# GrokImageCompression/Grok

Measured on NVIDIA H100. Metric: Mpixels/s encode+decode 8K RGB 12-bit HTJ2K; DWT HBM GB/s vs roofline, higher is better.
Workload: dtype i32

## Files before the change

grok_b200/csrc/b2k_internal.h:

```cpp
#pragma once
#include <stdint.h>
#include <stddef.h>
#include <atomic>
#include <functional>
#include <cuda_runtime.h>
#include "../../include/grok_b200.h"

#define B2K_WARPS_PER_CTA 4

struct DeviceOnce
{
  std::atomic<uint64_t> done{0};
  template <class F> void run(F&& f)
  {
    int dev = 0;
    cudaGetDevice(&dev);
    const uint64_t bit = 1ull << (dev & 63);
    if(!(done.load(std::memory_order_acquire) & bit))
    {
      f();
      done.fetch_or(bit, std::memory_order_release);
    }
  }
};
// ... 9 lines not shown
  int32_t shift[3];
  int32_t lo[3], hi[3];
  uint16_t nstrips, nsegs, strip_w, pairs_per_seg;
  uint8_t first_level;
  uint8_t comp0;
  uint8_t pad[2];
};

struct HtBlockDesc
{
  void* coef;
  uint32_t pitch;
  uint16_t w, h;
  uint8_t kmax;
  uint8_t irreversible;
  uint8_t mmsbs;
  uint8_t passes;
  float quant;
  uint32_t slot_cap;
  uint64_t slot_off;
  uint32_t length;
  uint32_t rec_off;
  uint32_t length2;
};
static_assert(sizeof(HtBlockDesc) == 56, "HtBlockDesc layout");

struct HtBlockOut
{
  uint32_t ms_len, mel_len, vlc_len, total;
};

void b2k_launch_dwt_fwd(const DwtLevelDesc* d_descs, int ndesc, int max_jobs, int nc, bool irreversible, cudaStream_t st);
void b2k_launch_dwt_inv(const DwtLevelDesc* d_descs, int ndesc, int max_jobs, int nc, bool irreversible, cudaStream_t st);
void b2k_launch_point_transform(const DwtLevelDesc* d_descs, int ndesc, uint32_t max_w, uint32_t max_h, int nc, bool irreversible,
                                bool forward, cudaStream_t st);
struct HtEncodeLimits
{
  uint32_t stage_words;
  uint32_t max_kmax;
};
uint32_t b2k_ht_encode_stage_words(uint32_t w);
void b2k_launch_ht_encode(const HtBlockDesc* d_blocks, HtBlockOut* d_out, uint8_t* d_scratch, uint32_t nblocks,
                          const HtEncodeLimits& lim, bool irreversible, cudaStream_t st);
void b2k_launch_ht_gather(const HtBlockDesc* d_blocks, const HtBlockOut* d_out, const uint64_t* d_offsets,
                          const uint8_t* d_scratch, uint8_t* d_bytes, uint32_t nblocks, uint64_t cap, cudaStream_t st);
void b2k_launch_scan_lengths(const HtBlockOut* d_out, uint64_t* d_offsets, uint32_t nblocks, cudaStream_t st);
void b2k_launch_ht_decode_refine(const HtBlockDesc* d_blocks, const uint8_t* d_bytes, const HtBlockOut* d_status,
                                 uint32_t nblocks, int stripe_causal, cudaStream_t st);
void b2k_launch_ht_decode(const HtBlockDesc* d_blocks, const uint8_t* d_bytes, uint32_t* d_recs, HtBlockOut* d_status,
                          uint32_t nblocks, uint32_t max_w, int* d_err, int irreversible, int any_refinement, cudaStream_t st);
void b2k_launch_ht_decode_vlc(const HtBlockDesc* d_blocks, const uint8_t* d_bytes, uint32_t* d_recs, HtBlockOut* d_status,
                              uint32_t nblocks, uint32_t max_w, cudaStream_t st);
void b2k_launch_ht_decode_magsgn(const HtBlockDesc* d_blocks, const uint8_t* d_bytes, const uint32_t* d_recs,
                                 const HtBlockOut* d_status, uint32_t nblocks, uint32_t max_w, int* d_err, int irreversible,
                                 int any_refinement, cudaStream_t st);
void b2k_launch_build_dec_desc(const HtBlockDesc* d_enc, const HtBlockOut* d_out, const uint64_t* d_offsets,
                               const float* d_dec_quant, HtBlockDesc* d_dec, uint32_t n, cudaStream_t st);
void b2k_launch_container_to_planes(const void* src, uint32_t spitch, uint32_t step, uint32_t sample_bytes, int32_t* const* dst, int nc,
                                    uint32_t dpitch, uint32_t w, uint32_t h, int sgnd, cudaStream_t st);
void b2k_launch_planes_to_container(const int32_t* const* src, int nc, uint32_t spitch, void* dst, uint32_t dpitch, uint32_t step,
                                    uint32_t sample_bytes, uint32_t w, uint32_t h, cudaStream_t st);
void b2k_count_launch(void);

struct b2k_host_rect
{
  const void* src;
// ... 11 lines not shown
```

grok_b200/csrc/dwt.cu:

```cuda
#include "b2k_internal.h"

namespace {

__device__ __noinline__ int mirror_rel_slow(int t, int n)
{
  if(n == 1)
    return 0;
  const int period = 2 * (n - 1);
  t %= period;
  if(t < 0)
    t += period;
  return t < n ? t : period - t;
}
__device__ __forceinline__ int mirror_rel(int t, int n)
{
  if((unsigned)t < (unsigned)n)
    return t;
  const int r = t < 0 ? -t : 2 * (n - 1) - t;
  if((unsigned)r < (unsigned)n)
    return r;
  return mirror_rel_slow(t, n);
}

__device__ __forceinline__ void load8_w32(const int32_t* __restrict__ row, int rel, int n, int (&v)[8])
// ... 11 lines not shown
#pragma unroll
    for(int i = 0; i < 8; ++i)
      v[i] = __ldg(row + mirror_rel(rel + i, n));
  }
}

__device__ __forceinline__ void load4_band(const int32_t* __restrict__ row, int k0, int kb0, int u0, int u1, int odd,
                                           int (&v)[4])
{
  const int ufirst = 2 * k0 + odd, ulast = ufirst + 6;
  const int32_t* p = row + (k0 - kb0);
  if(ufirst >= u0 && ulast < u1 && ((reinterpret_cast<uintptr_t>(p) & 15) == 0))
  {
    const int4 a = __ldg(reinterpret_cast<const int4*>(p));
    v[0] = a.x; v[1] = a.y; v[2] = a.z; v[3] = a.w;
  }
  else
  {
    const int n = u1 - u0;
#pragma unroll
    for(int i = 0; i < 4; ++i)
    {
      const int um = u0 + mirror_rel(ufirst + 2 * i - u0, n);
      v[i] = ((um & 1) == odd) ? __ldg(row + ((um >> 1) - kb0)) : 0;
    }
  }
}

struct Job
{
  int lane, ulane, jbeg, jend, wn, hn, nvalid;
  bool owner, need;
};
template <bool WHOLE>
__device__ __forceinline__ bool decode_job(const DwtLevelDesc& D, Job& J)
{
  J.lane = threadIdx.x & 31;
  const int job = blockIdx.x * B2K_WARPS_PER_CTA + (threadIdx.x >> 5);
  if(job >= (int)D.nstrips * (int)D.nsegs)
    return false;
  const int strip = job % D.nstrips, seg = job / D.nstrips;
  constexpr int halo = WHOLE ? 0 : 1;
  J.wn = D.u1 - D.u0;
  J.hn = D.v1 - D.v0;
  J.nvalid = D.strip_w >> 3;
  J.ulane = (D.u0 & ~7) + strip * (int)D.strip_w + (J.lane - halo) * 8;
  J.owner = J.lane >= halo && J.lane < J.nvalid + halo && J.ulane < D.u1;
  J.need = J.lane <= J.nvalid + halo && J.ulane < D.u1 + 8;
  const int jlo = D.v0 >> 1, jhi = (D.v1 - 1) >> 1;
  J.jbeg = jlo + seg * (int)D.pairs_per_seg;
  J.jend = min(J.jbeg + (int)D.pairs_per_seg, jhi + 1);
  return true;
}

template <int NC, int N>
__device__ __forceinline__ void rct_fwd(const DwtLevelDesc& D, int (&x)[NC][N])
{
#pragma unroll
  for(int i = 0; i < N; ++i)
  {
    if constexpr(NC == 3)
    {
      const int r = x[0][i] + D.shift[0], g = x[1][i] + D.shift[1], b = x[2][i] + D.shift[2];
      x[0][i] = ((g + g) + b + r) >> 2;
      x[1][i] = b - g;
      x[2][i] = r - g;
    }
    else
      x[0][i] += D.shift[0];
  }
}

template <int NC, int N>
__device__ __forceinline__ void ict_fwd(const DwtLevelDesc& D, const int (&x)[NC][N], float (&out)[NC][N])
{
  const float a_r = 0.299f, a_g = 0.587f, a_b = 0.114f;
  const float cb = __fdiv_rn(0.5f, __fsub_rn(1.0f, a_b)), cr = __fdiv_rn(0.5f, __fsub_rn(1.0f, a_r));
#pragma unroll
  for(int i = 0; i < N; ++i)
  {
    if constexpr(NC == 3)
    {
// ... 72 lines not shown
__device__ __forceinline__ void to_coeffs53(const DwtLevelDesc& D, int (&x)[NC][N])
{
  if(D.first_level)
    rct_fwd<NC, N>(D, x);
}

template <int NC>
__device__ __forceinline__ void to_coeffs97(const DwtLevelDesc& D, const int (&raw)[NC][8], float (&out)[NC][8])
{
  if(D.first_level)
    ict_fwd<NC>(D, raw, out);
  else
  {
#pragma unroll
    for(int c = 0; c < NC; ++c)
#pragma unroll
      for(int i = 0; i < 8; ++i)
        out[c][i] = __int_as_float(raw[c][i]);
  }
}

template <int NC>
__device__ __forceinline__ void fetch53(const DwtLevelDesc& D, const Job& J, int v, int (&out)[NC][8])
{
  fetch_int_rows<NC>(D, J, v, out);
  to_coeffs53<NC>(D, out);
}

struct GhostCol
{
  int col;
  int slot;
};
__device__ __forceinline__ GhostCol ghost_col(const DwtLevelDesc& D, const Job& J)
{
  const int x0 = J.ulane - 8 * J.lane;
  GhostCol G;
  G.slot = J.lane == 0 ? 0 : J.lane == 1 ? 1 : J.lane == 31 ? 2 : -1;
  const int x = J.lane == 0 ? x0 - 1 : J.lane == 1 ? x0 - 2 : J.lane == 31 ? x0 + 256 : J.ulane;
  G.col = mirror_rel(x - D.u0, J.wn);
  return G;
}
template <int NC>
__device__ __forceinline__ void fetch_ghost53(const DwtLevelDesc& D, const Job& J, const GhostCol& G, int v, int (&out)[NC][1])
{
  const int r = mirror_rel(v - D.v0, J.hn);
#pragma unroll
  for(int c = 0; c < NC; ++c)
    out[c][0] = __ldg(reinterpret_cast<const int32_t*>(D.in[c]) + (size_t)r * D.in_pitch + G.col);
  to_coeffs53<NC>(D, out);
}

template <int NC>
__device__ __forceinline__ void fetch97(const DwtLevelDesc& D, const Job& J, int v, float (&out)[NC][8])
{
  int raw[NC][8];
  fetch_int_rows<NC>(D, J, v, raw);
  to_coeffs97<NC>(D, raw, out);
}

struct BandGeom
{
  int x0l, x0h, y0l, y0h, snx, sny;
};
__device__ __forceinline__ BandGeom band_geom(const DwtLevelDesc& D)
{
  BandGeom g;
  g.x0l = (D.u0 + 1) >> 1;
  g.x0h = D.u0 >> 1;
  g.y0l = (D.v0 + 1) >> 1;
  g.y0h = D.v0 >> 1;
  g.snx = ((D.u1 + 1) >> 1) - g.x0l;
  g.sny = ((D.v1 + 1) >> 1) - g.y0l;
  return g;
}

struct StoreCtx
{
  unsigned mlo, mhi;
  bool vec_ll, vec_lo, vec_hi;
  int col_ll, col_lo, col_hi;
};
__device__ __forceinline__ StoreCtx store_ctx(const DwtLevelDesc& D, const Job& J, const BandGeom& g)
{
  StoreCtx s;
  s.mlo = s.mhi = 0;
  if(J.owner)
  {
#pragma unroll
    for(int i = 0; i < 4; ++i)
    {
      const int ue = J.ulane + 2 * i;
      if(ue >= D.u0 && ue < D.u1)
        s.mlo |= 1u << i;
      if(ue + 1 >= D.u0 && ue + 1 < D.u1)
        s.mhi |= 1u << i;
    }
  }
  const int k0 = J.ulane >> 1;
  s.col_ll = k0 - g.x0l;
  s.col_lo = k0 - g.x0l;
  s.col_hi = g.snx + k0 - g.x0h;
  const bool pitch_ok = ((D.ll_pitch | D.c_pitch) & 3u) == 0;
  s.vec_ll = pitch_ok && s.mlo == 0xF && (((reinterpret_cast<uintptr_t>(D.out_ll[0]) >> 2) + (unsigned)s.col_ll) & 3u) == 0;
  s.vec_lo = pitch_ok && s.mlo == 0xF && (((reinterpret_cast<uintptr_t>(D.out_c[0]) >> 2) + (unsigned)s.col_lo) & 3u) == 0;
  s.vec_hi = pitch_ok && s.mhi == 0xF && (((reinterpret_cast<uintptr_t>(D.out_c[0]) >> 2) + (unsigned)s.col_hi) & 3u) == 0;
  return s;
}
__device__ __forceinline__ void store4v(int32_t* __restrict__ p, const int (&v)[4], unsigned mask, bool vec)
{
  if(vec)
    *reinterpret_cast<int4*>(p) = make_int4(v[0], v[1], v[2], v[3]);
  else
  {
#pragma unroll
    for(int i = 0; i < 4; ++i)
      if(mask & (1u << i))
        p[i] = v[i];
  }
}
__device__ __forceinline__ void store_rows(const DwtLevelDesc& D, const BandGeom& g, const StoreCtx& S, int c, int j,
                                           bool vhigh, const int (&lo)[4], const int (&hi)[4])
{
  const int v = 2 * j + (vhigh ? 1 : 0);
  if(v < D.v0 || v >= D.v1 || (S.mlo | S.mhi) == 0)
    return;
  if(!vhigh)
  {
    const int r = j - g.y0l;
    store4v(reinterpret_cast<int32_t*>(D.out_ll[c]) + (r * (int)D.ll_pitch + S.col_ll), lo, S.mlo, S.vec_ll);
    store4v(reinterpret_cast<int32_t*>(D.out_c[c]) + (r * (int)D.c_pitch + S.col_hi), hi, S.mhi, S.vec_hi);
  }
  else
  {
    const int r = g.sny + j - g.y0h;
    int32_t* crow = reinterpret_cast<int32_t*>(D.out_c[c]) + r * (int)D.c_pitch;
    store4v(crow + S.col_lo, lo, S.mlo, S.vec_lo);
    store4v(crow + S.col_hi, hi, S.mhi, S.vec_hi);
  }
}

template <bool DEGEN = true>
__device__ __forceinline__ void hfwd53(const int (&r)[8], int g, int wn, int (&lo)[4], int (&hi)[4])
{
  const int lane = threadIdx.x & 31;
  const int g2 = __shfl_down_sync(0xffffffffu, g, 1);
  const int rn = __shfl_down_sync(0xffffffffu, r[0], 1);
  const int en = lane == 31 ? g : rn;
  hi[0] = r[1] - ((r[0] + r[2]) >> 1);
  hi[1] = r[3] - ((r[2] + r[4]) >> 1);
  hi[2] = r[5] - ((r[4] + r[6]) >> 1);
  hi[3] = r[7] - ((r[6] + en) >> 1);
  const int hp = __shfl_up_sync(0xffffffffu, hi[3], 1);
  const int dp = lane == 0 ? g - ((g2 + r[0]) >> 1) : hp;
  lo[0] = r[0] + ((dp + hi[0] + 2) >> 2);
  lo[1] = r[2] + ((hi[0] + hi[1] + 2) >> 2);
  lo[2] = r[4] + ((hi[1] + hi[2] + 2) >> 2);
  lo[3] = r[6] + ((hi[2] + hi[3] + 2) >> 2);
  if(DEGEN && wn == 1)
  {
#pragma unroll
    for(int i = 0; i < 4; ++i)
    {
      lo[i] = r[2 * i];
      hi[i] = r[2 * i + 1] << 1;
    }
  }
}

#define F97_ALPHA (-1.586134342f)
#define F97_BETA (-0.052980118f)
// ... 148 lines not shown
        mbar_fence_init();
      }
      __syncwarp();
    }
#pragma unroll
    for(int s = 0; s < DWT_STAGES - 1; ++s)
      refill(fill_bulk, fill_async, fill_side);
  }
  template <class Bulk, class Async, class Side = NoSideFill>
  __device__ __forceinline__ const uint8_t* acquire(int t, const Bulk& fill_bulk, const Async& fill_async,
                                                    const Side& fill_side = Side())
  {
    if(Stage::COOPERATIVE || bulk)
      __syncwarp();
    refill(fill_bulk, fill_async, fill_side);
    const int k = t - tfirst;
    if(bulk)
    {
      mbar_wait(bars + k % DWT_STAGES, (unsigned)((k / DWT_STAGES) & 1));
      if(Stage::GHOSTS)
        cp_async_wait<DWT_STAGES - 1>();
    }
    else
    {
      cp_async_wait<DWT_STAGES - 1>();
      if(Stage::COOPERATIVE)
        __syncwarp();
    }
    return slots + (size_t)(k % DWT_STAGES) * Stage::PAIRB;
  }
  __device__ __forceinline__ void drain() const { cp_async_wait<0>(); }
};

template <int NC, bool GHOSTS_ = false>
struct RowStage
{
  static constexpr int ROWB = 1024;
  static constexpr int BODYB = 2 * NC * ROWB;
  static constexpr bool GHOSTS = GHOSTS_;
  static constexpr int PAIRB = BODYB + (GHOSTS ? 2 * NC * 16 : 0);
  static constexpr bool COOPERATIVE = true;
  static __device__ __forceinline__ int swz(int k) { return k ^ ((k >> 3) & 1); }

  template <class MCol>
  static __device__ __forceinline__ void fill(uint8_t* stage, int which, const DwtLevelDesc& D, const Job& J, int v,
                                              bool fast, unsigned fastmask, const MCol& mcol)
  {
    const int r = mirror_rel(v - D.v0, J.hn);
    const int rel = J.ulane - D.u0;
#pragma unroll
    for(int c = 0; c < NC; ++c)
    {
      uint8_t* dst = stage + (which * NC + c) * ROWB;
      const int32_t* row = reinterpret_cast<const int32_t*>(D.in[c]) + (size_t)r * D.in_pitch;
      const int rel0 = rel - 8 * J.lane;
#pragma unroll
      for(int h = 0; h < 2; ++h)
      {
        const int k = J.lane + 32 * h;
        if((fastmask >> (k >> 1)) & 1u)
          cp_async16(dst + swz(k) * 16, row + rel0 + 4 * k);
      }
      if(J.need && !fast)
      {
        uint8_t* d0 = dst + swz(2 * J.lane) * 16;
        uint8_t* d1 = dst + swz(2 * J.lane + 1) * 16;
#pragma unroll
        for(int i = 0; i < 4; ++i)
        {
          cp_async4(d0 + 4 * i, row + mcol(i));
          cp_async4(d1 + 4 * i, row + mcol(4 + i));
        }
      }
    }
  }
  static __device__ __forceinline__ void fill_ghost(uint8_t* stage, int which, const DwtLevelDesc& D, const Job& J, int v,
                                                    const GhostCol& G)
  {
    static_assert(GHOSTS, "stage without ghost columns");
    const int r = mirror_rel(v - D.v0, J.hn);
#pragma unroll
    for(int c = 0; c < NC; ++c)
      if(G.slot >= 0)
        cp_async4(stage + BODYB + (which * NC + c) * 16 + 4 * G.slot,
                  reinterpret_cast<const int32_t*>(D.in[c]) + (size_t)r * D.in_pitch + G.col);
  }
  static __device__ __forceinline__ int2 ghost_at(const Job& J, const GhostCol& G)
  {
    return G.slot >= 0 ? make_int2(BODYB + 4 * G.slot, 16) : make_int2(32 * J.lane, ROWB);
  }
  static __device__ __forceinline__ void read_ghost(const uint8_t* stage, int which, int2 at, int (&out)[NC][1])
  {
#pragma unroll
    for(int c = 0; c < NC; ++c)
      out[c][0] = *reinterpret_cast<const int*>(stage + at.x + (which * NC + c) * at.y);
  }
  static __device__ __forceinline__ void fill_bulk(uint8_t* stage, int which, const DwtLevelDesc& D, const Job& J, int v, uint64_t* bar)
  {
    const int r = mirror_rel(v - D.v0, J.hn);
    const int rel0 = J.ulane - D.u0 - 8 * J.lane;
#pragma unroll
    for(int c = 0; c < NC; ++c)
      bulk_g2s(stage + (which * NC + c) * ROWB, reinterpret_cast<const int32_t*>(D.in[c]) + (size_t)r * D.in_pitch + rel0, ROWB, bar);
  }
  static __device__ __forceinline__ void read(const uint8_t* stage, int which, const Job& J, bool linear, int (&out)[NC][8])
  {
#pragma unroll
    for(int c = 0; c < NC; ++c)
    {
      const uint8_t* row = stage + (which * NC + c) * ROWB;
      int4 a, b;
      if(linear)
      {
        a = *reinterpret_cast<const int4*>(row + J.lane * 32);
        b = *reinterpret_cast<const int4*>(row + J.lane * 32 + 16);
      }
      else
      {
        a = *reinterpret_cast<const int4*>(row + swz(2 * J.lane) * 16);
        b = *reinterpret_cast<const int4*>(row + swz(2 * J.lane + 1) * 16);
      }
      out[c][0] = a.x; out[c][1] = a.y; out[c][2] = a.z; out[c][3] = a.w;
// ... 53 lines not shown
      int s[9], d[9];
#pragma unroll
      for(int i = 0; i < 9; ++i)
      {
        d[i] = O[c][i] - ((E[c][i] + E2[c][i]) >> 1);
        s[i] = E[c][i] + ((DP[c][i] + d[i] + 2) >> 2);
        if(J.hn == 1)
        {
          s[i] = E[c][i];
          d[i] = O[c][i] << 1;
        }
        DP[c][i] = d[i];
        E[c][i] = E2[c][i];
      }
      int s8[8], d8[8], lo[4], hi[4];
#pragma unroll
      for(int i = 0; i < 8; ++i)
      {
        s8[i] = s[i];
        d8[i] = d[i];
      }
      hfwd53<true>(s8, s[8], J.wn, lo, hi);
      store_rows(D, g, store_ctx(D, J, g), c, j, false, lo, hi);
      hfwd53<true>(d8, d[8], J.wn, lo, hi);
      store_rows(D, g, store_ctx(D, J, g), c, j, true, lo, hi);
    }
  }
}

template <int NC>
__global__ void __launch_bounds__(B2K_WARPS_PER_CTA * 32, 3) k_dwt53_fwd(const DwtLevelDesc* __restrict__ descs)
{
  extern __shared__ __align__(16) uint8_t smem_dwt[];
  typedef RowStage<NC, true> RS;
  const DwtLevelDesc D = descs[blockIdx.y];
  Job J;
  if(!decode_job<true>(D, J))
    return;
  if(J.hn == 1 || J.wn == 1)
  {
    fwd53_degenerate_job<NC>(descs + blockIdx.y, J);
    return;
  }
  const BandGeom g = band_geom(D);
  const StoreCtx SC = store_ctx(D, J, g);
  const bool fast = RS::lane_fast(D, J);
  const unsigned fastmask = __ballot_sync(0xffffffffu, fast);
  const GhostCol G = ghost_col(D, J);
  const int2 gat = RS::ghost_at(J, G);

  const int tfirst = J.jbeg - 1, tlast = J.jend - 1;
  WarpPipe<RS> pipe(smem_dwt, fastmask == 0xffffffffu, tfirst, tlast);
  auto fill_bulk = [&](uint8_t* st, int tf, uint64_t* bar) {
    RS::fill_bulk(st, 0, D, J, 2 * tf + 1, bar);
    RS::fill_bulk(st, 1, D, J, 2 * tf + 2, bar);
  };
  auto mcol = [&](int i) { return mirror_rel(J.ulane - D.u0 + i, J.wn); };
  auto fill_async = [&](uint8_t* st, int tf) {
    RS::fill(st, 0, D, J, 2 * tf + 1, fast, fastmask, mcol);
    RS::fill(st, 1, D, J, 2 * tf + 2, fast, fastmask, mcol);
  };
  auto fill_ghost = [&](uint8_t* st, int tf) {
    RS::fill_ghost(st, 0, D, J, 2 * tf + 1, G);
    RS::fill_ghost(st, 1, D, J, 2 * tf + 2, G);
  };
  pipe.prime(fill_bulk, fill_async, fill_ghost);
  int E[NC][8], DP[NC][8], gE[NC][1], gDP[NC];
// ... 20 lines not shown
    to_coeffs53<NC>(D, E2);
    to_coeffs53<NC>(D, gO);
    to_coeffs53<NC>(D, gE2);
    const bool emit = t >= J.jbeg;
#pragma unroll
    for(int c = 0; c < NC; ++c)
    {
      int s[8], d[8];
#pragma unroll
      for(int i = 0; i < 8; ++i)
      {
        d[i] = O[c][i] - ((E[c][i] + E2[c][i]) >> 1);
        s[i] = E[c][i] + ((DP[c][i] + d[i] + 2) >> 2);
        DP[c][i] = d[i];
        E[c][i] = E2[c][i];
      }
      const int gd = gO[c][0] - ((gE[c][0] + gE2[c][0]) >> 1);
      const int gs = gE[c][0] + ((gDP[c] + gd + 2) >> 2);
      gDP[c] = gd;
      gE[c][0] = gE2[c][0];
      if(emit)
      {
        int lo[4], hi[4];
        hfwd53<false>(s, gs, J.wn, lo, hi);
        store_rows(D, g, SC, c, t, false, lo, hi);
        hfwd53<false>(d, gd, J.wn, lo, hi);
        store_rows(D, g, SC, c, t, true, lo, hi);
      }
    }
  }
  pipe.drain();
}

template <int NC>
__device__ __noinline__ void fwd97_degenerate_job(const DwtLevelDesc* __restrict__ dptr, const Job J)
{
  const DwtLevelDesc& D = *dptr;
  const BandGeom g = band_geom(D);
  const float invK = (float)(1.0 / 1.230174105);
  const float deltaS = __fmul_rn(F97_DELTA, invK);

  float Ev[NC][8], D1[NC][8], S1[NC][8], D2[NC][8];
  fetch97<NC>(D, J, 2 * (J.jbeg - 2), Ev);
#pragma unroll
  for(int c = 0; c < NC; ++c)
#pragma unroll
    for(int i = 0; i < 8; ++i)
      D1[c][i] = S1[c][i] = D2[c][i] = 0.f;

  for(int t = J.jbeg - 2; t <= J.jend; ++t)
  {
    float O[NC][8], E2[NC][8];
    fetch97<NC>(D, J, 2 * t + 1, O);
    fetch97<NC>(D, J, 2 * t + 2, E2);
    const bool emit = (t - 1) >= J.jbeg;
#pragma unroll
    for(int c = 0; c < NC; ++c)
    {
      float lowrow[8], highrow[8];
#pragma unroll
      for(int i = 0; i < 8; ++i)
      {
        const float d1 = fmaf(Ev[c][i] + E2[c][i], F97_ALPHA, O[c][i]);
        const float s1 = fmaf(D1[c][i] + d1, F97_BETA, Ev[c][i]);
        const float d2 = __fmul_rn(fmaf(S1[c][i] + s1, F97_GAMMA, D1[c][i]), F97_K);
        const float s2 = __fmul_rn(fmaf(D2[c][i] + d2, deltaS, S1[c][i]), invK);
// ... 930 lines not shown
void b2k_launch_planes_to_container(const int32_t* const* src, int nc, uint32_t spitch, void* dst, uint32_t dpitch, uint32_t step,
                                    uint32_t sample_bytes, uint32_t w, uint32_t h, cudaStream_t st)
{
  if(!w || !h)
    return;
  CPtr4 P{};
  for(int c = 0; c < nc && c < 4; ++c)
    P.p[c] = src[c];
  switch(sample_bytes)
  {
    case 1: launch_planes_to_container<1>(P, nc, spitch, dst, dpitch, step, w, h, st); break;
    case 2: launch_planes_to_container<2>(P, nc, spitch, dst, dpitch, step, w, h, st); break;
    default: launch_planes_to_container<4>(P, nc, spitch, dst, dpitch, step, w, h, st); break;
  }
  b2k_count_launch();
}

template <class Stage, void (*KERNEL)(const DwtLevelDesc*)>
static void launch_dwt(dim3 grid, dim3 block, cudaStream_t st, const DwtLevelDesc* d)
{
  const size_t smem = WarpPipe<Stage>::SMEM_BYTES;
  static DeviceOnce once;
  once.run([&] { cudaFuncSetAttribute(KERNEL, cudaFuncAttributeMaxDynamicSharedMemorySize, (int)smem); });
  KERNEL<<<grid, block, smem, st>>>(d);
}

void b2k_launch_dwt_fwd(const DwtLevelDesc* d, int ndesc, int max_jobs, int nc, bool irreversible, cudaStream_t st)
{
  if(ndesc <= 0 || max_jobs <= 0)
    return;
  dim3 grid((max_jobs + B2K_WARPS_PER_CTA - 1) / B2K_WARPS_PER_CTA, ndesc), block(B2K_WARPS_PER_CTA * 32);
  if(!irreversible)
  {
    if(nc == 3) launch_dwt<RowStage<3, true>, k_dwt53_fwd<3>>(grid, block, st, d);
    else launch_dwt<RowStage<1, true>, k_dwt53_fwd<1>>(grid, block, st, d);
  }
  else
  {
    if(nc == 3) launch_dwt<RowStage<3>, k_dwt97_fwd<3>>(grid, block, st, d);
    else launch_dwt<RowStage<1>, k_dwt97_fwd<1>>(grid, block, st, d);
  }
  b2k_count_launch();
}

template <int NC, bool IRREV, bool FWD>
__global__ void k_point_transform(const DwtLevelDesc* __restrict__ descs, int ndesc)
{
  for(int di = blockIdx.z; di < ndesc; di += gridDim.z)
  {
  const DwtLevelDesc& D = descs[di];
  const int w = D.u1 - D.u0, h = D.v1 - D.v0;
  const int x = blockIdx.x * blockDim.x + threadIdx.x;
  if(x >= w)
    continue;
  for(int y = blockIdx.y; y < h; y += gridDim.y)
  {
  const size_t ii = (size_t)y * D.in_pitch + x, oi = (size_t)y * D.c_pitch + x;
  if(FWD)
  {
    int v[NC][1];
#pragma unroll
    for(int c = 0; c < NC; ++c)
      v[c][0] = static_cast<const int32_t*>(D.in[c])[ii];
    if(!IRREV)
    {
      rct_fwd<NC>(D, v);
#pragma unroll
      for(int c = 0; c < NC; ++c)
        static_cast<int32_t*>(D.out_c[c])[oi] = v[c][0];
    }
    else
    {
      float f[NC][1];
      ict_fwd<NC>(D, v, f);
// ... 70 lines not shown
```

grok_b200/csrc/engine.cu:

```cuda
#include <algorithm>
#include <atomic>
#include <chrono>
#include <cstdio>
#include <cstdlib>
#include <cstring>
#include <functional>
#include <map>
#include <mutex>
#include <unordered_map>
#include <string>
#include <vector>

#include "b2k_internal.h"
#include "geometry.h"

using namespace b2k;

static thread_local std::string g_err;
static std::atomic<uint64_t> g_launches{0};
static std::atomic<int> g_pack_policy{-1};
static std::atomic<int> g_last_pack[2]{{-1}, {-1}};
void b2k_count_launch(void) { g_launches.fetch_add(1, std::memory_order_relaxed); }

#define CUDA_TRY(expr)                                                                             \
// ... 179 lines not shown
#define cudaFree(p) dev_free((void*)(p))
#define cudaHostAlloc(p, n, flags) host_alloc_t((p), (n))
#define cudaFreeHost(p) host_free((void*)(p))

struct Planes
{
  int32_t* base = nullptr;
  uint32_t pitch = 0, rows = 0;
  uint32_t X0 = 0, Y0 = 0;
  int n = 0;
  size_t plane_elems() const { return (size_t)pitch * rows; }
  int32_t* at(int c, uint32_t x, uint32_t y) const { return base + (size_t)c * plane_elems() + (size_t)(y - Y0) * pitch + (x - X0); }
};

static int alloc_planes(Planes& p, int n, uint32_t cx0, uint32_t cy0, uint32_t cx1, uint32_t cy1)
{
  p.n = n;
  p.X0 = cx0 & ~31u;
  p.Y0 = cy0;
  p.pitch = ((cx1 - p.X0) + 31u + 32u) & ~31u;
  p.rows = (cy1 - cy0) + 2;
  CUDA_TRY(cudaMalloc(&p.base, (size_t)n * p.plane_elems() * sizeof(int32_t)));
  CUDA_TRY(cudaMemset(p.base, 0, (size_t)n * p.plane_elems() * sizeof(int32_t)));
  return 0;
}

struct LevelLaunch
{
  std::vector<DwtLevelDesc> descs;
  DwtLevelDesc* d_descs = nullptr;
  int nc = 1, max_jobs = 0;
  bool point = false;
  uint32_t max_w = 0, max_h = 0;
  uint64_t alg_bytes = 0;
  std::vector<uint32_t> tile_first;
};

#define B2K_MAX_CHUNKS 32
#define CEV(purpose, k) ((purpose) * (B2K_MAX_CHUNKS + 1) + (int)(k))

struct PackTuner
{
  int calls = 0;
  double best[2] = {1e30, 1e30};
  double recent = 0;
  int choice = -1;
  bool probing_other = false;
  bool next_mode()
  {
    if(choice < 0)
      return (calls & 1) == 0;
    probing_other = (calls % 64) == 63;
    return probing_other ? !choice : (choice != 0);
  }
  void record(bool packed, double ms)
  {
    ++calls;
    if(choice < 0)
    {
      if(calls > 1 || !packed)
        best[packed ? 1 : 0] = std::min(best[packed ? 1 : 0], ms);
      if(calls >= 6)
      {
        choice = best[1] < best[0] ? 1 : 0;
        recent = best[choice];
      }
// ... 137 lines not shown
  b2k_host_set_threads(n);
  g_pack_policy.store(n < 0 ? -1 : n == 0 ? 0 : 1);
  return b2k_host_threads();
}

extern "C" int32_t b2k_host_pack_last(int32_t decode) { return g_last_pack[decode ? 1 : 0].load(); }

extern "C" void b2k_host_free(void* p)
{
  if(p)
    cudaFreeHost(p);
}

extern "C" int64_t b2k_enumerate(const b2k_coding* cp, uint32_t tile_mod, uint32_t tile_rem, b2k_block* out, uint64_t cap)
{
  if(!cp || tile_mod == 0)
    return -1;
  if(const char* why = unsupported_reason(*cp))
  {
    g_err = why;
    return -1;
  }
  const TileGrid g = tile_grid(*cp);
  const std::vector<BandQuant> q = band_quant(*cp);
  std::vector<b2k_block> v;
  for(uint32_t t = 0; t < g.nx * g.ny; ++t)
    if(t % tile_mod == tile_rem)
      enumerate_tile_blocks(*cp, t, tile_rect(*cp, g, t), q, v);
  for(uint64_t i = 0; i < v.size() && i < cap; ++i)
    out[i] = v[i];
  return (int64_t)v.size();
}

static void fill_strips(DwtLevelDesc& d, int pairs_per_seg, bool whole_warp)
{
  const int span = d.u1 - (d.u0 & ~7);
  const int nstrips = std::max(1, whole_warp ? (span + 255) / 256 : (span + 239) / 240);
  int sw = whole_warp ? 256 : (span + nstrips - 1) / nstrips;
  sw = (sw + 7) & ~7;
  d.nstrips = (uint16_t)nstrips;
  d.strip_w = (uint16_t)sw;
  const int npairs = ((d.v1 - 1) >> 1) - (d.v0 >> 1) + 1;
  d.pairs_per_seg = (uint16_t)pairs_per_seg;
  d.nsegs = (uint16_t)((npairs + pairs_per_seg - 1) / pairs_per_seg);
}

static int upload_descs(LevelLaunch& L)
{
  L.max_jobs = 0;
  for(const DwtLevelDesc& d : L.descs)
    L.max_jobs = std::max(L.max_jobs, (int)d.nstrips * (int)d.nsegs);
  if(L.descs.empty())
    return 0;
  CUDA_TRY(cudaMalloc(&L.d_descs, L.descs.size() * sizeof(DwtLevelDesc)));
  CUDA_TRY(cudaMemcpy(L.d_descs, L.descs.data(), L.descs.size() * sizeof(DwtLevelDesc), cudaMemcpyHostToDevice));
  return 0;
}

static int build_dwt_plan(b2k_device_job* J)
{
  const b2k_coding& cp = J->cp;
  const int L = cp.numres - 1;
  const int ncomp = cp.numcomps;
  const int pairs53 = 32, pairs97 = 32;
  const int P = cp.irreversible ? pairs97 : pairs53;
  const int32_t dc = cp.sgnd ? 0 : -(1 << (cp.prec - 1));
  const int32_t lo = cp.sgnd ? -(1 << (cp.prec - 1)) : 0, hi = cp.sgnd ? (1 << (cp.prec - 1)) - 1 : (1 << cp.prec) - 1;

  if(L == 0)
  {
    for(int dir = 0; dir < 2; ++dir)
    {
      std::vector<LevelLaunch>& out = dir == 0 ? J->fwd : J->inv;
      LevelLaunch mctL, sglL;
      mctL.nc = 3;
// ... 16 lines not shown
          d.first_level = 1;
          d.comp0 = (uint8_t)c;
          for(int k = 0; k < nc; ++k)
          {
            d.in[k] = J->img.at(c + k, tc.x0, tc.y0);
            d.in_pitch = J->img.pitch;
            d.out_c[k] = J->coef.at(c + k, tc.x0, tc.y0);
            d.out_ll[k] = d.out_c[k];
            d.c_pitch = d.ll_pitch = J->coef.pitch;
            d.shift[k] = dc;
            d.lo[k] = lo;
            d.hi[k] = hi;
          }
          LL.descs.push_back(d);
          LL.max_w = std::max(LL.max_w, tc.w());
          LL.max_h = std::max(LL.max_h, tc.h());
          LL.alg_bytes += (uint64_t)tc.w() * tc.h() * nc * 8;
          c += nc;
        }
      }
      mctL.tile_first.push_back((uint32_t)mctL.descs.size());
      sglL.tile_first.push_back((uint32_t)sglL.descs.size());
      if(!mctL.descs.empty()) out.push_back(std::move(mctL));
      if(!sglL.descs.empty()) out.push_back(std::move(sglL));
      for(LevelLaunch& Lh : out)
      {
        Lh.max_jobs = 1;
        if(upload_descs(Lh))
          return -1;
      }
    }
    return 0;
  }
  for(int dir = 0; dir < 2; ++dir)
  {
    std::vector<LevelLaunch>& out = dir == 0 ? J->fwd : J->inv;
    for(int lvl = 1; lvl <= L; ++lvl)
    {
      const int resno = cp.numres - lvl;
      LevelLaunch mctL, sglL;
      mctL.nc = 3;
      sglL.nc = 1;
      for(size_t ti = 0; ti < J->tiles.size(); ++ti)
      {
        mctL.tile_first.push_back((uint32_t)mctL.descs.size());
        sglL.tile_first.push_back((uint32_t)sglL.descs.size());
        const Rect tc = J->tile_rects[ti];
        const Rect r = resolution_rect(tc, cp.numres, resno);
        if(r.empty())
          continue;
        for(int c = 0; c < ncomp;)
        {
          const bool group = (lvl == 1 && cp.mct && c == 0);
          const int nc = group ? 3 : 1;
          DwtLevelDesc d{};
          d.u0 = (int32_t)r.x0; d.v0 = (int32_t)r.y0; d.u1 = (int32_t)r.x1; d.v1 = (int32_t)r.y1;
          d.first_level = lvl == 1;
          d.comp0 = (uint8_t)c;
          const uint32_t llx = (r.x0 + 1) >> 1, lly = (r.y0 + 1) >> 1;
          for(int k = 0; k < nc; ++k)
          {
            const int cc = c + k;
            const Planes& fine = (lvl == 1) ? J->img : J->ll[(lvl - 1) & 1];
            d.in[k] = fine.at(cc, r.x0, r.y0);
            d.in_pitch = fine.pitch;
            d.out_c[k] = J->coef.at(cc, tc.x0, tc.y0);
            d.c_pitch = J->coef.pitch;
            if(lvl == L)
            {
              d.out_ll[k] = d.out_c[k];
              d.ll_pitch = J->coef.pitch;
            }
            else
            {
              const Planes& coarse = J->ll[lvl & 1];
              d.out_ll[k] = coarse.at(cc, llx, lly);
              d.ll_pitch = coarse.pitch;
            }
            d.shift[k] = dc;
            d.lo[k] = lo;
            d.hi[k] = hi;
          }
          fill_strips(d, P, !cp.irreversible);
          (group ? mctL : sglL).descs.push_back(d);
          const uint64_t samples = (uint64_t)r.w() * r.h() * nc;
          (group ? mctL : sglL).alg_bytes += samples * 8;
          c += nc;
        }
      }
      mctL.tile_first.push_back((uint32_t)mctL.descs.size());
      sglL.tile_first.push_back((uint32_t)sglL.descs.size());
      for(LevelLaunch* LL : {&mctL, &sglL})
      {
        int Pl = P;
        auto jobs = [&] {
          uint64_t n = 0;
          for(const DwtLevelDesc& d : LL->descs)
            n += (uint64_t)d.nstrips * d.nsegs;
          return n;
        };
        while(!LL->descs.empty() && Pl > 8 && jobs() < 3552)
        {
          Pl >>= 1;
          for(DwtLevelDesc& d : LL->descs)
            fill_strips(d, Pl, !cp.irreversible);
        }
      }
      if(dir == 0)
      {
        if(!mctL.descs.empty()) out.push_back(std::move(mctL));
        if(!sglL.descs.empty()) out.push_back(std::move(sglL));
      }
      else
      {
        if(!sglL.descs.empty()) out.insert(out.begin(), std::move(sglL));
        if(!mctL.descs.empty()) out.insert(out.begin(), std::move(mctL));
      }
    }
    for(LevelLaunch& Lh : out)
      if(upload_descs(Lh))
        return -1;
  }
  return 0;
}

static uint32_t slot_capacity(uint32_t w, uint32_t h, uint32_t kmax)
{
  const uint64_t samples = (uint64_t)w * h, quads = (uint64_t)((w + 1) / 2) * ((h + 1) / 2);
  const uint64_t ms = (samples * (kmax + 2) + 6) / 7 + 16;
  const uint64_t vlc = (quads * 15 + 6) / 7 + 16;
  return (uint32_t)((ms + vlc + 256 + 15) & ~15ull);
}

static int build_block_plan(b2k_device_job* J)
{
  const b2k_coding& cp = J->cp;
  J->blocks.clear();
  for(size_t ti = 0; ti < J->tiles.size(); ++ti)
// ... 613 lines not shown
  CUDA_TRY(cudaStreamWaitEvent(st, J->chunk_ev[CEV(0, k)], 0));
  return 0;
}

static int download_chunk(b2k_device_job* J, const Transport& T, size_t k, cudaStream_t st, cudaStream_t cs)
{
  const size_t t0 = J->chunk_tile[k], t1 = J->chunk_tile[k + 1];
  if(T.user.device)
    return device_convert(J, T.user, false, st, t0, t1, T.window);
  if(T.staged && device_convert(J, T.stage, false, st, t0, t1, T.window))
    return -1;
  CUDA_TRY(cudaEventRecord(J->chunk_ev[CEV(0, k)], st));
  if(T.ring)
    return 0;
  CUDA_TRY(cudaStreamWaitEvent(cs, J->chunk_ev[CEV(0, k)], 0));
  return copy_runs(J, T.user, T.staged ? T.stage : plane_container(J->img), cs, t0, t1, T.window);
}

static int enqueue_forward(b2k_device_job* J, cudaStream_t st, bool time_level1, size_t t0 = 0, size_t t1 = (size_t)-1,
                           cudaEvent_t l1_begin = nullptr, cudaEvent_t l1_end = nullptr)
{
  if(!l1_begin) l1_begin = J->ev[4];
  if(!l1_end) l1_end = J->ev[5];
  t1 = std::min(t1, J->tiles.size());
  bool first = true;
  for(size_t li = 0; li < J->fwd.size(); ++li)
  {
    LevelLaunch& L = J->fwd[li];
    const uint32_t d0 = L.tile_first[t0], d1 = L.tile_first[t1];
    if(first && time_level1)
      CUDA_TRY(cudaEventRecord(l1_begin, st));
    if(d1 > d0 && L.point)
      b2k_launch_point_transform(L.d_descs + d0, (int)(d1 - d0), L.max_w, L.max_h, L.nc, J->cp.irreversible, true, st);
    else if(d1 > d0)
      b2k_launch_dwt_fwd(L.d_descs + d0, (int)(d1 - d0), L.max_jobs, L.nc, J->cp.irreversible, st);
    if(first && time_level1)
    {
      CUDA_TRY(cudaEventRecord(l1_end, st));
      J->level1_alg_bytes = L.alg_bytes;
    }
    first = false;
  }
  CUDA_TRY(cudaGetLastError());
  return 0;
}

static int enqueue_inverse(b2k_device_job* J, cudaStream_t st, size_t t0 = 0, size_t t1 = (size_t)-1)
{
  t1 = std::min(t1, J->tiles.size());
  for(size_t li = 0; li < J->inv.size(); ++li)
  {
    LevelLaunch& L = J->inv[li];
    const uint32_t d0 = L.tile_first[t0], d1 = L.tile_first[t1];
    if(d1 > d0 && L.point)
      b2k_launch_point_transform(L.d_descs + d0, (int)(d1 - d0), L.max_w, L.max_h, L.nc, J->cp.irreversible, false, st);
    else if(d1 > d0)
      b2k_launch_dwt_inv(L.d_descs + d0, (int)(d1 - d0), L.max_jobs, L.nc, J->cp.irreversible, st);
  }
  CUDA_TRY(cudaGetLastError());
  return 0;
}

static int enqueue_t1_blocks(b2k_device_job* J, cudaStream_t st, size_t t0, size_t t1)
{
  t1 = std::min(t1, J->tiles.size());
  const uint32_t b0 = J->coded_first[t0], b1 = J->coded_first[t1];
// ... 1095 lines not shown
```

Before: 14140.

## Fuse first two forward 5/3 DWT levels into one kernel

Adds a kernel that computes DWT level 1 and then, from the LL rows held in registers, level 2 in the same pass. The level-1 LL plane is therefore never written to or re-read from HBM, and one launch is removed. The engine uses this fused kernel for reversible encodes with at least two levels and skips the separate level-2 launch. It needs wider ghost columns, more registers (launch bounds reduced to 2 CTAs per SM), and halves the pairs per segment, which may lower occupancy.

Result: faster. 14580 (median of 6 runs) (+3.1%).

```diff
diff --git a/grok_b200/csrc/b2k_internal.h b/grok_b200/csrc/b2k_internal.h
--- a/grok_b200/csrc/b2k_internal.h
+++ b/grok_b200/csrc/b2k_internal.h
@@ -65,6 +65,7 @@
 
 void b2k_launch_dwt_fwd(const DwtLevelDesc* d_descs, int ndesc, int max_jobs, int nc, bool irreversible, cudaStream_t st);
 void b2k_launch_dwt_inv(const DwtLevelDesc* d_descs, int ndesc, int max_jobs, int nc, bool irreversible, cudaStream_t st);
+void b2k_launch_dwt53_fwd12(const DwtLevelDesc* d_descs, int ndesc, int max_jobs, int nc, cudaStream_t st);
 void b2k_launch_point_transform(const DwtLevelDesc* d_descs, int ndesc, uint32_t max_w, uint32_t max_h, int nc, bool irreversible,
                                 bool forward, cudaStream_t st);
 struct HtEncodeLimits
diff --git a/grok_b200/csrc/dwt.cu b/grok_b200/csrc/dwt.cu
--- a/grok_b200/csrc/dwt.cu
+++ b/grok_b200/csrc/dwt.cu
@@ -67,7 +67,7 @@
   int lane, ulane, jbeg, jend, wn, hn, nvalid;
   bool owner, need;
 };
-template <bool WHOLE>
+template <bool WHOLE, bool FUSED = false>
 __device__ __forceinline__ bool decode_job(const DwtLevelDesc& D, Job& J)
 {
   J.lane = threadIdx.x & 31;
@@ -82,7 +82,8 @@
   J.ulane = (D.u0 & ~7) + strip * (int)D.strip_w + (J.lane - halo) * 8;
   J.owner = J.lane >= halo && J.lane < J.nvalid + halo && J.ulane < D.u1;
   J.need = J.lane <= J.nvalid + halo && J.ulane < D.u1 + 8;
-  const int jlo = D.v0 >> 1, jhi = (D.v1 - 1) >> 1;
+  const int v0 = FUSED ? (D.v0 + 1) >> 1 : D.v0, v1 = FUSED ? (D.v1 + 1) >> 1 : D.v1;
+  const int jlo = v0 >> 1, jhi = (v1 - 1) >> 1;
   J.jbeg = jlo + seg * (int)D.pairs_per_seg;
   J.jend = min(J.jbeg + (int)D.pairs_per_seg, jhi + 1);
   return true;
@@ -221,12 +222,22 @@
   int col;
   int slot;
 };
+template <bool FUSED = false>
 __device__ __forceinline__ GhostCol ghost_col(const DwtLevelDesc& D, const Job& J)
 {
   const int x0 = J.ulane - 8 * J.lane;
   GhostCol G;
-  G.slot = J.lane == 0 ? 0 : J.lane == 1 ? 1 : J.lane == 31 ? 2 : -1;
-  const int x = J.lane == 0 ? x0 - 1 : J.lane == 1 ? x0 - 2 : J.lane == 31 ? x0 + 256 : J.ulane;
+  int x;
+  if(FUSED)
+  {
+    G.slot = J.lane <= 5 ? J.lane : J.lane >= 29 ? 37 - J.lane : -1;
+    x = J.lane <= 5 ? x0 - 1 - J.lane : J.lane >= 29 ? x0 + 287 - J.lane : J.ulane;
+  }
+  else
+  {
+    G.slot = J.lane == 0 ? 0 : J.lane == 1 ? 1 : J.lane == 31 ? 2 : -1;
+    x = J.lane == 0 ? x0 - 1 : J.lane == 1 ? x0 - 2 : J.lane == 31 ? x0 + 256 : J.ulane;
+  }
   G.col = mirror_rel(x - D.u0, J.wn);
   return G;
 }
@@ -251,18 +262,22 @@
 struct BandGeom
 {
   int x0l, x0h, y0l, y0h, snx, sny;
+  int v0, v1;
 };
-__device__ __forceinline__ BandGeom band_geom(const DwtLevelDesc& D)
+__device__ __forceinline__ BandGeom band_geom_of(int u0, int v0, int u1, int v1)
 {
   BandGeom g;
-  g.x0l = (D.u0 + 1) >> 1;
-  g.x0h = D.u0 >> 1;
-  g.y0l = (D.v0 + 1) >> 1;
-  g.y0h = D.v0 >> 1;
-  g.snx = ((D.u1 + 1) >> 1) - g.x0l;
-  g.sny = ((D.v1 + 1) >> 1) - g.y0l;
+  g.x0l = (u0 + 1) >> 1;
+  g.x0h = u0 >> 1;
+  g.y0l = (v0 + 1) >> 1;
+  g.y0h = v0 >> 1;
+  g.snx = ((u1 + 1) >> 1) - g.x0l;
+  g.sny = ((v1 + 1) >> 1) - g.y0l;
+  g.v0 = v0;
+  g.v1 = v1;
   return g;
 }
+__device__ __forceinline__ BandGeom band_geom(const DwtLevelDesc& D) { return band_geom_of(D.u0, D.v0, D.u1, D.v1); }
 
 struct StoreCtx
 {
@@ -296,36 +311,67 @@
   s.vec_hi = pitch_ok && s.mhi == 0xF && (((reinterpret_cast<uintptr_t>(D.out_c[0]) >> 2) + (unsigned)s.col_hi) & 3u) == 0;
   return s;
 }
-__device__ __forceinline__ void store4v(int32_t* __restrict__ p, const int (&v)[4], unsigned mask, bool vec)
+__device__ __forceinline__ StoreCtx store_ctx_ll1(const DwtLevelDesc& D, const Job& J, const BandGeom& g2, int a, int b)
+{
+  StoreCtx s;
+  s.mlo = s.mhi = 0;
+  const int kb = J.ulane >> 1;
+#pragma unroll
+  for(int i = 0; i < 2; ++i)
+  {
+    if(kb + 2 * i >= a && kb + 2 * i < b)
+      s.mlo |= 1u << i;
+    if(kb + 2 * i + 1 >= a && kb + 2 * i + 1 < b)
+      s.mhi |= 1u << i;
+  }
+  const int k0 = kb >> 1;
+  s.col_ll = k0 - g2.x0l;
+  s.col_lo = k0 - g2.x0l;
+  s.col_hi = g2.snx + k0 - g2.x0h;
+  const bool pitch_ok = ((D.ll_pitch | D.c_pitch) & 3u) == 0;
+  s.vec_ll = pitch_ok && s.mlo == 3 && (((reinterpret_cast<uintptr_t>(D.out_ll[0]) >> 2) + (unsigned)s.col_ll) & 1u) == 0;
+  s.vec_lo = pitch_ok && s.mlo == 3 && (((reinterpret_cast<uintptr_t>(D.out_c[0]) >> 2) + (unsigned)s.col_lo) & 1u) == 0;
+  s.vec_hi = pitch_ok && s.mhi == 3 && (((reinterpret_cast<uintptr_t>(D.out_c[0]) >> 2) + (unsigned)s.col_hi) & 1u) == 0;
+  return s;
+}
+template <int N>
+__device__ __forceinline__ void storev(int32_t* __restrict__ p, const int (&v)[N], unsigned mask, bool vec)
 {
   if(vec)
-    *reinterpret_cast<int4*>(p) = make_int4(v[0], v[1], v[2], v[3]);
+  {
+    if constexpr(N == 4)
+      *reinterpret_cast<int4*>(p) = make_int4(v[0], v[1], v[2], v[3]);
+    else
+      *reinterpret_cast<int2*>(p) = make_int2(v[0], v[1]);
+  }
   else
   {
 #pragma unroll
-    for(int i = 0; i < 4; ++i)
+    for(int i = 0; i < N; ++i)
       if(mask & (1u << i))
         p[i] = v[i];
   }
 }
+template <int N = 4, bool LL = true>
 __device__ __forceinline__ void store_rows(const DwtLevelDesc& D, const BandGeom& g, const StoreCtx& S, int c, int j,
-                                           bool vhigh, const int (&lo)[4], const int (&hi)[4])
+                                           bool vhigh, const int (&lo)[N], const int (&hi)[N])
 {
   const int v = 2 * j + (vhigh ? 1 : 0);
-  if(v < D.v0 || v >= D.v1 || (S.mlo | S.mhi) == 0)
+  if(v < g.v0 || v >= g.v1 || (S.mlo | S.mhi) == 0)
     return;
   if(!vhigh)
   {
     const int r = j - g.y0l;
-    store4v(reinterpret_cast<int32_t*>(D.out_ll[c]) + (r * (int)D.ll_pitch + S.col_ll), lo, S.mlo, S.vec_ll);
-    store4v(reinterpret_cast<int32_t*>(D.out_c[c]) + (r * (int)D.c_pitch + S.col_hi), hi, S.mhi, S.vec_hi);
+    if(LL)
+      storev<N>(reinterpret_cast<int32_t*>(D.out_ll[c]) + (r * (int)D.ll_pitch + S.col_ll), lo, S.mlo, S.vec_ll);
+    storev<N>(reinterpret_cast<int32_t*>(D.out_c[c]) + (r * (int)D.c_pitch + S.col_hi), hi, S.mhi, S.vec_hi);
   }
   else
   {
     const int r = g.sny + j - g.y0h;
     int32_t* crow = reinterpret_cast<int32_t*>(D.out_c[c]) + r * (int)D.c_pitch;
-    store4v(crow + S.col_lo, lo, S.mlo, S.vec_lo);
-    store4v(crow + S.col_hi, hi, S.mhi, S.vec_hi);
+    storev<N>(crow + S.col_lo, lo, S.mlo, S.vec_lo);
+    storev<N>(crow + S.col_hi, hi, S.mhi, S.vec_hi);
   }
 }
 
@@ -540,13 +586,14 @@
   __device__ __forceinline__ void drain() const { cp_async_wait<0>(); }
 };
 
-template <int NC, bool GHOSTS_ = false>
+template <int NC, int GHOSTW = 0>
 struct RowStage
 {
   static constexpr int ROWB = 1024;
   static constexpr int BODYB = 2 * NC * ROWB;
-  static constexpr bool GHOSTS = GHOSTS_;
-  static constexpr int PAIRB = BODYB + (GHOSTS ? 2 * NC * 16 : 0);
+  static constexpr bool GHOSTS = GHOSTW > 0;
+  static constexpr int GROUPB = 4 * GHOSTW;
+  static constexpr int PAIRB = (BODYB + 2 * NC * GROUPB + 15) & ~15;
   static constexpr bool COOPERATIVE = true;
   static __device__ __forceinline__ int swz(int k) { return k ^ ((k >> 3) & 1); }
 
@@ -590,12 +637,12 @@
 #pragma unroll
     for(int c = 0; c < NC; ++c)
       if(G.slot >= 0)
-        cp_async4(stage + BODYB + (which * NC + c) * 16 + 4 * G.slot,
+        cp_async4(stage + BODYB + (which * NC + c) * GROUPB + 4 * G.slot,
                   reinterpret_cast<const int32_t*>(D.in[c]) + (size_t)r * D.in_pitch + G.col);
   }
   static __device__ __forceinline__ int2 ghost_at(const Job& J, const GhostCol& G)
   {
-    return G.slot >= 0 ? make_int2(BODYB + 4 * G.slot, 16) : make_int2(32 * J.lane, ROWB);
+    return G.slot >= 0 ? make_int2(BODYB + 4 * G.slot, GROUPB) : make_int2(32 * J.lane, ROWB);
   }
   static __device__ __forceinline__ void read_ghost(const uint8_t* stage, int which, int2 at, int (&out)[NC][1])
   {
@@ -715,7 +762,7 @@
 __global__ void __launch_bounds__(B2K_WARPS_PER_CTA * 32, 3) k_dwt53_fwd(const DwtLevelDesc* __restrict__ descs)
 {
   extern __shared__ __align__(16) uint8_t smem_dwt[];
-  typedef RowStage<NC, true> RS;
+  typedef RowStage<NC, 3> RS;
   const DwtLevelDesc D = descs[blockIdx.y];
   Job J;
   if(!decode_job<true>(D, J))
@@ -802,6 +849,179 @@
   pipe.drain();
 }
 
+__device__ __forceinline__ int ll1_ghost(const int (&s)[8], int gs)
+{
+  const int lane = threadIdx.x & 31;
+  int sh[5];
+#pragma unroll
+  for(int k = 1; k <= 4; ++k)
+    sh[k] = __shfl_sync(0xffffffffu, gs, lane == 31 ? 31 - k : (lane + k) & 31);
+  const int m2 = lane == 31 ? s[6] : lane == 0 ? sh[3] : sh[4];
+  const int m1 = lane == 31 ? s[7] : lane == 0 ? sh[2] : sh[3];
+  const int c0 = lane == 31 ? gs : lane == 0 ? sh[1] : sh[2];
+  const int p1 = lane == 31 ? sh[1] : lane == 0 ? gs : sh[1];
+  const int p2 = lane == 31 ? sh[2] : lane == 0 ? s[0] : gs;
+  const int dm = m1 - ((m2 + c0) >> 1), dp = p1 - ((c0 + p2) >> 1);
+  return c0 + ((dm + dp + 2) >> 2);
+}
+
+__device__ __forceinline__ void hfwd53_ll1(const int (&e)[5], int kb, int a, int b, int (&lo)[2], int (&hi)[2])
+{
+  const int lane = threadIdx.x & 31;
+  const int g2 = __shfl_down_sync(0xffffffffu, e[4], 1);
+  const int rn = __shfl_down_sync(0xffffffffu, e[0], 1);
+  const int en = lane == 31 ? e[4] : rn;
+  int l = kb + 1 == a ? e[2] : e[0], r = kb + 2 == b ? e[0] : e[2];
+  hi[0] = e[1] - ((l + r) >> 1);
+  l = kb + 3 == a ? en : e[2];
+  r = kb + 4 == b ? e[2] : en;
+  hi[1] = e[3] - ((l + r) >> 1);
+  const int hp = __shfl_up_sync(0xffffffffu, hi[1], 1);
+  const int dp = lane == 0 ? e[4] - ((g2 + e[0]) >> 1) : hp;
+  l = kb == a ? hi[0] : dp;
+  r = kb + 1 == b ? dp : hi[0];
+  lo[0] = e[0] + ((l + r + 2) >> 2);
+  l = kb + 2 == a ? hi[1] : hi[0];
+  r = kb + 3 == b ? hi[0] : hi[1];
+  lo[1] = e[2] + ((l + r + 2) >> 2);
+}
+
+template <int NC>
+__global__ void __launch_bounds__(B2K_WARPS_PER_CTA * 32, 2) k_dwt53_fwd12(const DwtLevelDesc* __restrict__ descs)
+{
+  extern __shared__ __align__(16) uint8_t smem_dwt[];
+  typedef RowStage<NC, 9> RS;
+  const DwtLevelDesc D = descs[blockIdx.y];
+  Job J;
+  if(!decode_job<true, true>(D, J))
+    return;
+  const BandGeom g = band_geom(D);
+  const int a = g.x0l, b = g.x0l + g.snx, A = g.y0l, B = g.y0l + g.sny;
+  const BandGeom g2 = band_geom_of(a, A, b, B);
+  const StoreCtx SC = store_ctx(D, J, g);
+  const StoreCtx SC2 = store_ctx_ll1(D, J, g2, a, b);
+  const bool fast = RS::lane_fast(D, J);
+  const unsigned fastmask = __ballot_sync(0xffffffffu, fast);
+  const GhostCol G = ghost_col<true>(D, J);
+  const int2 gat = RS::ghost_at(J, G);
+  const int kb = J.ulane >> 1;
+
+  const int tfirst = 2 * J.jbeg - 3, tlast = 2 * J.jend;
+  const int t1lo = J.jbeg == (A >> 1) ? (D.v0 >> 1) : 2 * J.jbeg, t1hi = 2 * J.jend;
+  WarpPipe<RS> pipe(smem_dwt, fastmask == 0xffffffffu, tfirst, tlast);
+  auto fill_bulk = [&](uint8_t* st, int tf, uint64_t* bar) {
+    RS::fill_bulk(st, 0, D, J, 2 * tf + 1, bar);
+    RS::fill_bulk(st, 1, D, J, 2 * tf + 2, bar);
+  };
+  auto mcol = [&](int i) { return mirror_rel(J.ulane - D.u0 + i, J.wn); };
+  auto fill_async = [&](uint8_t* st, int tf) {
+    RS::fill(st, 0, D, J, 2 * tf + 1, fast, fastmask, mcol);
+    RS::fill(st, 1, D, J, 2 * tf + 2, fast, fastmask, mcol);
+  };
+  auto fill_ghost = [&](uint8_t* st, int tf) {
+    RS::fill_ghost(st, 0, D, J, 2 * tf + 1, G);
+    RS::fill_ghost(st, 1, D, J, 2 * tf + 2, G);
+  };
+  pipe.prime(fill_bulk, fill_async, fill_ghost);
+  int E[NC][8], DP[NC][8], gE[NC][1], gDP[NC];
+  fetch53<NC>(D, J, 2 * tfirst, E);
+  fetch_ghost53<NC>(D, J, G, 2 * tfirst, gE);
+  int E2[NC][5], O2[NC][5], D2[NC][5];
+#pragma unroll
+  for(int c = 0; c < NC; ++c)
+  {
+#pragma unroll
+    for(int i = 0; i < 8; ++i)
+      DP[c][i] = 0;
+    gDP[c] = 0;
+#pragma unroll
+    for(int i = 0; i < 5; ++i)
+      E2[c][i] = O2[c][i] = D2[c][i] = 0;
+  }
+
+  for(int t = tfirst; t <= tlast; ++t)
+  {
+    const uint8_t* st = pipe.acquire(t, fill_bulk, fill_async, fill_ghost);
+    int O[NC][8], En[NC][8], gO[NC][1], gEn[NC][1];
+    RS::read(st, 0, J, pipe.bulk, O);
+    RS::read(st, 1, J, pipe.bulk, En);
+    RS::read_ghost(st, 0, gat, gO);
+    RS::read_ghost(st, 1, gat, gEn);
+    to_coeffs53<NC>(D, O);
+    to_coeffs53<NC>(D, En);
+    to_coeffs53<NC>(D, gO);
+    to_coeffs53<NC>(D, gEn);
+    const bool emit = t >= t1lo && t < t1hi;
+    const int t2 = (t >> 1) - 1;
+    const bool step2 = (t & 1) == 0 && t > tfirst + 1, emit2 = t2 >= J.jbeg;
+    const bool top = 2 * t2 < A, bot = 2 * t2 + 2 >= B, first = 2 * t2 <= A, last = 2 * t2 + 1 >= B;
+#pragma unroll
+    for(int c = 0; c < NC; ++c)
+    {
+      int s[8], d[8];
+#pragma unroll
+      for(int i = 0; i < 8; ++i)
+      {
+        d[i] = O[c][i] - ((E[c][i] + En[c][i]) >> 1);
+        s[i] = E[c][i] + ((DP[c][i] + d[i] + 2) >> 2);
+        DP[c][i] = d[i];
+        E[c][i] = En[c][i];
+      }
+      const int gd = gO[c][0] - ((gE[c][0] + gEn[c][0]) >> 1);
+      const int gs = gE[c][0] + ((gDP[c] + gd + 2) >> 2);
+      gDP[c] = gd;
+      gE[c][0] = gEn[c][0];
+      int row[5], lo[4], hi[4];
+      hfwd53<false>(s, gs, J.wn, lo, hi);
+      row[4] = ll1_ghost(s, gs);
+      if(emit)
+      {
+        store_rows<4, false>(D, g, SC, c, t, false, lo, hi);
+        int dlo[4], dhi[4];
+        hfwd53<false>(d, gd, J.wn, dlo, dhi);
+        store_rows(D, g, SC, c, t, true, dlo, dhi);
+      }
+#pragma unroll
+      for(int i = 0; i < 4; ++i)
+        row[i] = lo[i];
+      if(t & 1)
+      {
+#pragma unroll
+        for(int i = 0; i < 5; ++i)
+          O2[c][i] = row[i];
+        continue;
+      }
+      if(step2)
+      {
+        int s2[5], d2[5];
+#pragma unroll
+        for(int i = 0; i < 5; ++i)
+        {
+          const int e = top ? row[i] : E2[c][i];
+          const int en = bot ? e : row[i];
+          d2[i] = O2[c][i] - ((e + en) >> 1);
+          const int dl = first ? d2[i] : D2[c][i];
+          const int dr = last ? dl : d2[i];
+          s2[i] = e + ((dl + dr + 2) >> 2);
+          D2[c][i] = d2[i];
+        }
+        if(emit2)
+        {
+          int l2[2], h2[2];
+          hfwd53_ll1(s2, kb, a, b, l2, h2);
+          store_rows<2>(D, g2, SC2, c, t2, false, l2, h2);
+          hfwd53_ll1(d2, kb, a, b, l2, h2);
+          store_rows<2>(D, g2, SC2, c, t2, true, l2, h2);
+        }
+      }
+#pragma unroll
+      for(int i = 0; i < 5; ++i)
+        E2[c][i] = row[i];
+    }
+  }
+  pipe.drain();
+}
+
 template <int NC>
 __device__ __noinline__ void fwd97_degenerate_job(const DwtLevelDesc* __restrict__ dptr, const Job J)
 {
@@ -1798,14 +2018,24 @@
   dim3 grid((max_jobs + B2K_WARPS_PER_CTA - 1) / B2K_WARPS_PER_CTA, ndesc), block(B2K_WARPS_PER_CTA * 32);
   if(!irreversible)
   {
-    if(nc == 3) launch_dwt<RowStage<3, true>, k_dwt53_fwd<3>>(grid, block, st, d);
-    else launch_dwt<RowStage<1, true>, k_dwt53_fwd<1>>(grid, block, st, d);
+    if(nc == 3) launch_dwt<RowStage<3, 3>, k_dwt53_fwd<3>>(grid, block, st, d);
+    else launch_dwt<RowStage<1, 3>, k_dwt53_fwd<1>>(grid, block, st, d);
   }
   else
   {
     if(nc == 3) launch_dwt<RowStage<3>, k_dwt97_fwd<3>>(grid, block, st, d);
     else launch_dwt<RowStage<1>, k_dwt97_fwd<1>>(grid, block, st, d);
   }
+  b2k_count_launch();
+}
+
+void b2k_launch_dwt53_fwd12(const DwtLevelDesc* d, int ndesc, int max_jobs, int nc, cudaStream_t st)
+{
+  if(ndesc <= 0 || max_jobs <= 0)
+    return;
+  dim3 grid((max_jobs + B2K_WARPS_PER_CTA - 1) / B2K_WARPS_PER_CTA, ndesc), block(B2K_WARPS_PER_CTA * 32);
+  if(nc == 3) launch_dwt<RowStage<3, 9>, k_dwt53_fwd12<3>>(grid, block, st, d);
+  else launch_dwt<RowStage<1, 9>, k_dwt53_fwd12<1>>(grid, block, st, d);
   b2k_count_launch();
 }
 
diff --git a/grok_b200/csrc/engine.cu b/grok_b200/csrc/engine.cu
--- a/grok_b200/csrc/engine.cu
+++ b/grok_b200/csrc/engine.cu
@@ -235,6 +235,7 @@
   int nc = 1, max_jobs = 0;
   bool point = false;
   uint32_t max_w = 0, max_h = 0;
+  bool fused = false;
   uint64_t alg_bytes = 0;
   std::vector<uint32_t> tile_first;
 };
@@ -438,7 +439,7 @@
   return (int64_t)v.size();
 }
 
-static void fill_strips(DwtLevelDesc& d, int pairs_per_seg, bool whole_warp)
+static void fill_strips(DwtLevelDesc& d, int pairs_per_seg, bool whole_warp, bool fused = false)
 {
   const int span = d.u1 - (d.u0 & ~7);
   const int nstrips = std::max(1, whole_warp ? (span + 255) / 256 : (span + 239) / 240);
@@ -446,7 +447,8 @@
   sw = (sw + 7) & ~7;
   d.nstrips = (uint16_t)nstrips;
   d.strip_w = (uint16_t)sw;
-  const int npairs = ((d.v1 - 1) >> 1) - (d.v0 >> 1) + 1;
+  const int v0 = fused ? (d.v0 + 1) >> 1 : d.v0, v1 = fused ? (d.v1 + 1) >> 1 : d.v1;
+  const int npairs = ((v1 - 1) >> 1) - (v0 >> 1) + 1;
   d.pairs_per_seg = (uint16_t)pairs_per_seg;
   d.nsegs = (uint16_t)((npairs + pairs_per_seg - 1) / pairs_per_seg);
 }
@@ -529,15 +531,25 @@
     }
     return 0;
   }
+  bool fuse12 = !cp.irreversible && L >= 2;
+  for(size_t ti = 0; ti < J->tiles.size() && fuse12; ++ti)
+  {
+    const Rect r2 = resolution_rect(J->tile_rects[ti], cp.numres, cp.numres - 2);
+    fuse12 = J->tile_rects[ti].empty() || (r2.w() >= 2 && r2.h() >= 2);
+  }
   for(int dir = 0; dir < 2; ++dir)
   {
     std::vector<LevelLaunch>& out = dir == 0 ? J->fwd : J->inv;
     for(int lvl = 1; lvl <= L; ++lvl)
     {
+      const bool fused = dir == 0 && fuse12 && lvl == 1;
+      if(dir == 0 && fuse12 && lvl == 2)
+        continue;
       const int resno = cp.numres - lvl;
       LevelLaunch mctL, sglL;
       mctL.nc = 3;
       sglL.nc = 1;
+      mctL.fused = sglL.fused = fused;
       for(size_t ti = 0; ti < J->tiles.size(); ++ti)
       {
         mctL.tile_first.push_back((uint32_t)mctL.descs.size());
@@ -563,7 +575,14 @@
             d.in_pitch = fine.pitch;
             d.out_c[k] = J->coef.at(cc, tc.x0, tc.y0);
             d.c_pitch = J->coef.pitch;
-            if(lvl == L)
+            if(fused)
+            {
+              const Rect r2 = resolution_rect(tc, cp.numres, resno - 1);
+              const Planes& coarse = L == 2 ? J->coef : J->ll[0];
+              d.out_ll[k] = L == 2 ? J->coef.at(cc, tc.x0, tc.y0) : coarse.at(cc, (r2.x0 + 1) >> 1, (r2.y0 + 1) >> 1);
+              d.ll_pitch = coarse.pitch;
+            }
+            else if(lvl == L)
             {
               d.out_ll[k] = d.out_c[k];
               d.ll_pitch = J->coef.pitch;
@@ -578,7 +597,7 @@
             d.lo[k] = lo;
             d.hi[k] = hi;
           }
-          fill_strips(d, P, !cp.irreversible);
+          fill_strips(d, fused ? P / 2 : P, !cp.irreversible, fused);
           (group ? mctL : sglL).descs.push_back(d);
           const uint64_t samples = (uint64_t)r.w() * r.h() * nc;
           (group ? mctL : sglL).alg_bytes += samples * 8;
@@ -589,7 +608,7 @@
       sglL.tile_first.push_back((uint32_t)sglL.descs.size());
       for(LevelLaunch* LL : {&mctL, &sglL})
       {
-        int Pl = P;
+        int Pl = fused ? P / 2 : P;
         auto jobs = [&] {
           uint64_t n = 0;
           for(const DwtLevelDesc& d : LL->descs)
@@ -600,7 +619,7 @@
         {
           Pl >>= 1;
           for(DwtLevelDesc& d : LL->descs)
-            fill_strips(d, Pl, !cp.irreversible);
+            fill_strips(d, Pl, !cp.irreversible, fused);
         }
       }
       if(dir == 0)
@@ -1280,6 +1299,8 @@
       CUDA_TRY(cudaEventRecord(l1_begin, st));
     if(d1 > d0 && L.point)
       b2k_launch_point_transform(L.d_descs + d0, (int)(d1 - d0), L.max_w, L.max_h, L.nc, J->cp.irreversible, true, st);
+    else if(d1 > d0 && L.fused)
+      b2k_launch_dwt53_fwd12(L.d_descs + d0, (int)(d1 - d0), L.max_jobs, L.nc, st);
     else if(d1 > d0)
       b2k_launch_dwt_fwd(L.d_descs + d0, (int)(d1 - d0), L.max_jobs, L.nc, J->cp.irreversible, st);
     if(first && time_level1)
```
